# angelvillar96/STLPose

Hardware: AMD Instinct MI355X
Metric: images/sec/GPU HRNet-W32 384x288 train step; PCKh@0.5 parity (higher is better)
Workload: dtype f16/bf16; 1 GPU; HRNet-W32 384x288 bs=32/GPU train step (fwd+MSE+bwd+Adam), random-init weights; global_batch=32, parallelism=dp1

## Files before the change

### stlpose_amd/capi.py

```python
from __future__ import annotations

import ctypes as C
import os

import torch

from .cheader import Header

_HERE = os.path.dirname(os.path.abspath(__file__))
LIB_PATH = os.environ.get("STLPOSE_HIP_LIB") or os.path.join(_HERE, "libstlpose_hip.so")
INCLUDE = os.path.join(_HERE, "..", "include")
vp, i32, i64, f32 = C.c_void_p, C.c_int32, C.c_int64, C.c_float

CLASS_NAMES = {
    "stl_src": "Src", "stl_conv": "Conv", "stl_wgrad": "Wgrad", "stl_wgrad_io": "WgradIO", "stl_wgrad_group": "WgradGroup",
    "stl_term": "Term", "stl_fuse": "Fuse", "stl_fuse_bwd": "FuseBwd", "stl_upbwd": "UpBwd", "stl_wprep": "WPrep", "stl_slab": "Slab",
    "stl_bnrec": "BNRec", "stl_reduce_range": "ReduceRange", "stl_bn_range": "BNRange", "stl_patch": "Patch",
    "stl_patch_bwd": "PatchBwd", "stl_head": "Head", "stl_head_bwd": "HeadBwd", "stl_op": "Op", "StlDetImage": "DetImage",
    "StlDetPointwise": "DetPointwise", "StlDetTerm": "DetTerm", "StlDetFuse": "DetFuse", "StlDetPointwise16": "DetPointwise16",
    "StlDetPointwiseBwd": "DetPointwiseBwd", "StlDetPointwise16Bwd": "DetPointwise16Bwd"}
DEVICE_RECORDS = ("stl_wprep", "stl_slab", "stl_bnrec", "StlDetImage")

HEADER = Header(os.path.join(INCLUDE, "stlpose_hip.h"), CLASS_NAMES, DEVICE_RECORDS)
if set(HEADER.structs) != set(CLASS_NAMES):
    raise ImportError(f"capi.CLASS_NAMES and the structs of include/stlpose_hip.h differ: {sorted(set(HEADER.structs) ^ set(CLASS_NAMES))}")
globals().update({name[len("STL_"):]: value for name, value in HEADER.constants.items()})
globals().update({cls.__name__: cls for cls in HEADER.structs.values()})
SIGNATURES, RESTYPES = HEADER.signatures, HEADER.restypes
INT64_FUNCS = tuple(n for n, r in RESTYPES.items() if r is C.c_int64)
STRING_FUNCS = tuple(n for n, r in RESTYPES.items() if r is C.c_char_p)
DEBUG_SIGNATURES = Header(os.path.join(INCLUDE, "stlpose_hip_debug.h")).signatures
DETECTIONS = Header(os.path.join(INCLUDE, "stlpose_hip_detections.h"))

DTYPES = {F32: (4, torch.float32), BF16: (2, torch.bfloat16), F16: (2, torch.float16)}


def dt2(grad_dtype: int, fwd_dtype: int) -> int:
    return grad_dtype | ((fwd_dtype if fwd_dtype != grad_dtype else 0) << 8)


MIXED = dt2(BF16, F16)
POSE_APPROACH = {"all_kpts": POSE_ALL_KPTS, "full_body": POSE_FULL_BODY, "upper_body": POSE_UPPER_BODY}
POSE_DIM = {"all_kpts": 34, "full_body": 26, "upper_body": 18}
POSE_METHOD = {"euclidean": POSE_EUCLIDEAN, "cosine": POSE_COSINE, "manhattan": POSE_MANHATTAN, "confidence": POSE_CONFIDENCE,
               "oks": POSE_OKS, "l2sq": POSE_L2SQ, "cos_normalised": POSE_COS_NORMALISED}
POSE_PEN = {"zero_coord": POSE_PEN_ZERO_COORD, "none": POSE_PEN_NONE, "mean": POSE_PEN_MEAN, "max": POSE_PEN_MAX}
POSE_SUM_ORDER = {"numpy": POSE_SUM_NUMPY, "reference": POSE_SUM_SERIAL}
# ... 7 lines not shown

def lib() -> C.CDLL:
    global _lib
    if _lib is None:
        if not os.path.exists(LIB_PATH):
            raise RuntimeError(
                f"{LIB_PATH} not found: build it with `python -m stlpose_amd.build` "
                "(hipcc --offload-arch=gfx950). There is no CPU fallback for the product path.")
        l = C.CDLL(LIB_PATH)
        for name, args in SIGNATURES.items():
            fn = getattr(l, name)
            fn.argtypes, fn.restype = args, RESTYPES[name]
        for name, args in DETECTIONS.signatures.items():
            fn = getattr(l, name)
            fn.argtypes, fn.restype = args, DETECTIONS.restypes[name]
        for name, args in DEBUG_SIGNATURES.items():
            if hasattr(l, name):
                getattr(l, name).argtypes, getattr(l, name).restype = args, C.c_int
        _lib = l
    return _lib


def check(rc: int, what: str = "") -> None:
    if rc != 0:
        raise RuntimeError(f"stlpose_hip {what}: {lib().stl_last_error().decode()}")


def call(name: str, *args) -> None:
    check(getattr(lib(), name)(*args), name)
```

### stlpose_amd/csrc/elementwise.hip

```cpp
#include "common.cuh"

namespace {

template <typename T>
__device__ __forceinline__ void load8(const void* base, size_t elem, float* f) {
    if constexpr (sizeof(T) == 2) {
        unpack<T>(ldg16((const char*)base + elem * 2), f);
    } else {
        unpack<float>(ldg16((const char*)base + elem * 4), f);
        unpack<float>(ldg16((const char*)base + elem * 4 + 16), f + 4);
    }
}
template <typename T>
__device__ __forceinline__ void store8(void* base, size_t elem, const float* f) {
    if constexpr (sizeof(T) == 2) {
        stg16((char*)base + elem * 2, pack<T>(f));
    } else {
        stg16((char*)base + elem * 4, pack<float>(f));
        stg16((char*)base + elem * 4 + 16, pack<float>(f + 4));
    }
}

template <int NS>
__device__ __forceinline__ void flush_sets(float (*acc)[8], float* red, int C, int VPC, double* const* dst,
// ... 517 lines not shown

__global__ __launch_bounds__(256) void mse_kernel(const float* o, const float* t, const float* tw, float* dout,
                                                  double* partial, size_t n, int HW, float gs) {
    double acc = 0.0;
    for (size_t i = (size_t)blockIdx.x * 256 + threadIdx.x; i < n; i += (size_t)gridDim.x * 256) {
        const float w = tw[i / HW];
        const float d = (o[i] - t[i]) * w;
        acc += (double)d * (double)d;
        if (dout) dout[i] = d * w * gs;
    }
    __shared__ double sred[4];
    acc = wave_sum_d(acc);
    if ((threadIdx.x & 63) == 0) sred[threadIdx.x >> 6] = acc;
    __syncthreads();
    if (threadIdx.x == 0) partial[blockIdx.x] = sred[0] + sred[1] + sred[2] + sred[3];
}

__global__ __launch_bounds__(256) void sum_partials_kernel(const double* partial, int n, double scale, float* out, int accumulate) {
    double acc = 0.0;
    for (int i = threadIdx.x; i < n; i += 256) acc += partial[i];
    __shared__ double sred[4];
    acc = wave_sum_d(acc);
    if ((threadIdx.x & 63) == 0) sred[threadIdx.x >> 6] = acc;
    __syncthreads();
    if (threadIdx.x == 0) {
        const double s = (sred[0] + sred[1] + sred[2] + sred[3]) * scale;
        out[0] = (float)((accumulate ? (double)out[0] : 0.0) + s);
    }
}

// ... 89 lines not shown
    uint2 u;
    u.x = (uint32_t)__builtin_bit_cast(unsigned short, v[0]) | ((uint32_t)__builtin_bit_cast(unsigned short, v[1]) << 16);
    u.y = (uint32_t)__builtin_bit_cast(unsigned short, v[2]) | ((uint32_t)__builtin_bit_cast(unsigned short, v[3]) << 16);
    *reinterpret_cast<uint2*>(dst) = u;
}
__device__ __forceinline__ void store_vec4(f16* dst, const f16* v) {
    uint2 u;
    u.x = (uint32_t)__builtin_bit_cast(unsigned short, v[0]) | ((uint32_t)__builtin_bit_cast(unsigned short, v[1]) << 16);
    u.y = (uint32_t)__builtin_bit_cast(unsigned short, v[2]) | ((uint32_t)__builtin_bit_cast(unsigned short, v[3]) << 16);
    *reinterpret_cast<uint2*>(dst) = u;
}
__device__ __forceinline__ void store_vec4(float* dst, const float* v) {
    *reinterpret_cast<float4*>(dst) = make_float4(v[0], v[1], v[2], v[3]);
}

template <typename T, typename TF = T>
__global__ __launch_bounds__(256) void weight_prep_kernel(const float* master, T* wk, const stl_wprep* tab, int n, int blk_base) {
    static_assert(sizeof(T) == sizeof(TF), "both layouts live in one buffer of equal-width elements");
    TF* wkf = reinterpret_cast<TF*>(wk);
    const int bx = blockIdx.x + blk_base;
    const int ei = find_entry(&tab[0].blk0, sizeof(stl_wprep) / 4, n, bx);
    const stl_wprep e = tab[ei];
    const int t = e.ks * e.ks;
    const int64_t tot = (int64_t)e.Co * e.Ci * t;
    const int64_t base = (int64_t)(bx - e.blk0) * 1024;
    if (!e.patch && (e.Ci & 3) == 0 && (e.Co & 3) == 0 && t <= 9 && e.Cip == e.Ci && (e.fwd_off & 3) == 0 && (e.bwd_off < 0 || (e.bwd_off & 3) == 0)) {
        __shared__ float st[32 * (32 * 9 + 1)];
        const int pitch = 32 * t + 1;
        const int tci = (e.Ci + 31) >> 5, ntiles = ((e.Co + 31) >> 5) * tci;
        const int nblk = (int)((tot + 1023) / 1024);
        const float* src0 = master + e.src_off;
        for (int tile = bx - e.blk0; tile < ntiles; tile += nblk) {
            const int co0 = (tile / tci) * 32, ci0 = (tile % tci) * 32;
            const int nco = min(32, e.Co - co0), nci = min(32, e.Ci - ci0), seg = nci * t;
            __syncthreads();
            if (((e.src_off & 3) | (int)((uintptr_t)master & 15)) == 0) {
                const int nv = seg >> 2, ntask = nco * nv;
                float4 buf[9];
#pragma unroll
                for (int u = 0; u < 9; ++u) {
                    const int i = threadIdx.x + u * 256;
                    const bool ok = i < ntask;
                    const int r = ok ? i / nv : 0, q = ok ? i - r * nv : 0;
                    buf[u] = *reinterpret_cast<const float4*>(src0 + ((int64_t)(co0 + r) * e.Ci + ci0) * t + 4 * q);
                }
#pragma unroll
                for (int u = 0; u < 9; ++u) {
                    const int i = threadIdx.x + u * 256;
                    if (i < ntask) {
                        const int r = i / nv, q = i - r * nv;
                        float* d = st + r * pitch + 4 * q;
// ... 22 lines not shown
                for (int i = threadIdx.x; i < nci * t * p4; i += 256) {
                    const int row = p4 == 8 ? i >> 3 : i / p4, r4 = (i - row * p4) * 4;
                    const int c = t == 9 ? row / 9 : (t == 1 ? row : row / t), tapf = row - c * t;
#pragma unroll
                    for (int j = 0; j < 4; ++j) v[j] = (T)st[(r4 + j) * pitch + c * t + (t - 1 - tapf)];
                    store_vec4(wk + e.bwd_off + ((int64_t)(ci0 + c) * t + tapf) * e.Co + co0 + r4, v);
                }
            }
        }
        return;
    }
    for (int r = 0; r < 4; ++r) {
        const int64_t i = base + r * 256 + threadIdx.x;
        if (i >= tot) return;
        const int co = (int)(i / (e.Ci * t)), rem = (int)(i - (int64_t)co * e.Ci * t), ci = rem / t, tap = rem - ci * t;
        const float v = master[e.src_off + i];
        if (e.patch)
            wkf[e.fwd_off + (int64_t)co * e.Cip + tap * e.Ci + ci] = (TF)v;
        else
            wkf[e.fwd_off + ((int64_t)co * t + tap) * e.Cip + ci] = (TF)v;
        if (e.bwd_off >= 0) {
            if (e.patch)
                wk[e.bwd_off + (int64_t)(tap * e.Ci + ci) * e.Co + co] = (T)v;
            else
                wk[e.bwd_off + ((int64_t)ci * t + (t - 1 - tap)) * e.Co + co] = (T)v;
        }
    }
}

__global__ __launch_bounds__(256) void reduce_slabs_kernel(const float* partials, float* grads, const stl_slab* tab, int n, int blk_base) {
    const int bx = blockIdx.x + blk_base;
    const int ei = find_entry(&tab[0].blk0, sizeof(stl_slab) / 4, n, bx);
    const stl_slab e = tab[ei];
    const int t = e.ks * e.ks;
    const int64_t tot = (int64_t)e.Co * e.Ci * t;
    const int tk = e.patch ? 1 : t, cik = e.patch ? e.Cip : e.Ci;
    const int64_t slab = e.pad ? (int64_t)e.pad : (int64_t)e.Co * tk * cik;
    const int64_t base = (int64_t)(bx - e.blk0) * 1024;
    if (!e.patch && (e.Ci & 3) == 0) {
        const int64_t j = base + 4 * threadIdx.x;
        if (j >= tot) return;
        const float* src = partials + e.part_off + j;
// ... 80 lines not shown
            r1 += rstats[e.stats_off + (int64_t)k * 2 * e.C + c];
            r2 += rstats[e.stats_off + (int64_t)k * 2 * e.C + e.C + c];
        }
        grads[e.param_off + c] = (float)r2;
        grads[e.param_off + e.C + c] = (float)r1;
    }
}

__global__ void inc_step_kernel(int32_t* step, const int32_t* overflow) {
    const int t = step[0] < 0 ? -step[0] - 1 : step[0];
    step[0] = (overflow && overflow[0] != 0x7fffffff) ? -t - 1 : t + 1;
}

__global__ __launch_bounds__(256) void adam_kernel(float* p, const float* g, float* m, float* v, int64_t n,
                                                   const float* hyper, const int32_t* step) {
    const float lr = hyper[0], b1 = hyper[1], b2 = hyper[2], eps = hyper[3], wd = hyper[4], gs = hyper[7];
    const int t = step[0];
    if (t < 0) return;
    const float bc1 = 1.f - powf(b1, (float)t), bc2 = 1.f - powf(b2, (float)t);
    const float step_size = lr / bc1, isq2 = 1.f / sqrtf(bc2);
    for (int64_t i = (int64_t)blockIdx.x * 256 + threadIdx.x; i < n; i += (int64_t)gridDim.x * 256) {
        float gi = g[i] * gs;
        if (!(fabsf(gi) <= 3.4e38f)) continue;
        const float pi = p[i];
        if (wd != 0.f) gi = fmaf(wd, pi, gi);
        const float mi = b1 * m[i] + (1.f - b1) * gi;
        const float vi = b2 * v[i] + (1.f - b2) * gi * gi;
        m[i] = mi, v[i] = vi;
        p[i] = pi - step_size * mi / (sqrtf(vi) * isq2 + eps);
    }
}

__global__ __launch_bounds__(256) void sgd_kernel(float* p, const float* g, float* mom, int64_t n, const float* hyper,
                                                  const int32_t* step) {
    const float lr = hyper[0], wd = hyper[4], mu = hyper[5], nest = hyper[6], gs = hyper[7];
    if (step[0] < 0) return;
    const bool first = step[0] <= 1;
    for (int64_t i = (int64_t)blockIdx.x * 256 + threadIdx.x; i < n; i += (int64_t)gridDim.x * 256) {
        float gi = g[i] * gs;
        if (!(fabsf(gi) <= 3.4e38f)) continue;
        const float pi = p[i];
        if (wd != 0.f) gi = fmaf(wd, pi, gi);
        if (mu != 0.f) {
            const float b = first ? gi : mu * mom[i] + gi;
// ... 437 lines not shown
    STL_LAUNCH(sum_partials_kernel, dim3(1), dim3(256), 0, ST, partial, n, scale, out, accumulate);
    STL_LAUNCH_CHECK("sum_partials");
    return 0;
}

extern "C" int stl_mse_loss(const float* out, const float* target, const float* tweight, float* dout, double* partial,
                            int nblk, float* loss, int B, int J, int HW, float gscale, void* stream) {
    STL_CHECK(out && target && tweight && partial && nblk >= 1, "mse: null pointer");
    const size_t n = (size_t)B * J * HW;
    STL_LAUNCH(mse_kernel, dim3(nblk), dim3(256), 0, ST, out, target, tweight, dout, partial, n, HW, gscale / (float)n);
    STL_LAUNCH_CHECK("mse_loss");
    if (!loss) return 0;
    return stl_sum_partials(partial, nblk, 0.5 / (double)n, loss, 0, stream);
}

extern "C" int stl_heatmap_argmax(const float* hm, int32_t* idx, float* maxval, float* preds, int BJ, int H, int W, void* stream) {
    if (BJ == 0) return 0;
    STL_CHECK(hm && maxval && preds && H > 0 && W > 0, "argmax: bad args");
    STL_LAUNCH(argmax_kernel, dim3(BJ), dim3(256), 0, ST, hm, idx, maxval, preds, H, W);
    STL_LAUNCH_CHECK("heatmap_argmax");
    return 0;
}

extern "C" int stl_final_preds(const float* hm, const float* center, const float* scale, float* preds, float* maxval, int B,
                               int J, int H, int W, void* stream) {
    if (B * J == 0) return 0;
    STL_LAUNCH(final_preds_kernel, dim3(B * J), dim3(256), 0, ST, hm, center, scale, preds, maxval, J, H, W);
    STL_LAUNCH_CHECK("final_preds");
    return 0;
}
// ... 57 lines not shown
    return 0;
}

extern "C" int stl_bn_param_grads(const double* rstats, float* grads, const stl_bnrec* tab, int n, void* stream) {
    if (n == 0) return 0;
    STL_LAUNCH(bn_param_grads_kernel, dim3(n), dim3(256), 0, ST, rstats, grads, tab);
    STL_LAUNCH_CHECK("bn_param_grads");
    return 0;
}

extern "C" int stl_adam_step(float* p, const float* g, float* m, float* v, int64_t n, const float* hyper, int32_t* step, const int32_t* overflow,
                             void* stream) {
    STL_LAUNCH(inc_step_kernel, dim3(1), dim3(1), 0, ST, step, overflow);
    STL_LAUNCH(adam_kernel, dim3(nblocks_for((size_t)n, 256, 4096)), dim3(256), 0, ST, p, g, m, v, n, hyper, step);
    STL_LAUNCH_CHECK("adam_step");
    return 0;
}

extern "C" int stl_sgd_step(float* p, const float* g, float* mom, int64_t n, const float* hyper, int32_t* step, const int32_t* overflow, void* stream) {
    STL_LAUNCH(inc_step_kernel, dim3(1), dim3(1), 0, ST, step, overflow);
    STL_LAUNCH(sgd_kernel, dim3(nblocks_for((size_t)n, 256, 4096)), dim3(256), 0, ST, p, g, mom, n, hyper, step);
    STL_LAUNCH_CHECK("sgd_step");
    return 0;
}

__global__ __launch_bounds__(256) void gaussian_targets_kernel(const float* __restrict__ joints, const float* __restrict__ vis,
                                                               float* __restrict__ target, float* __restrict__ tw, int BJ, int Hh,
                                                               int Wh, double sx, double sy, float sigma) {
    const size_t total = (size_t)BJ * Hh * Wh;
    const float r = sigma * 3.f;
// ... 140 lines not shown
```

### stlpose_amd/engine.py

```python
from __future__ import annotations

import bisect
import ctypes as C
import math
import os
from dataclasses import dataclass, field
from typing import Dict, List, NamedTuple, Optional, Tuple, Union

import torch

from . import capi
from .arch import Arch, Registry, registry, walk

EPS = 1e-5
MOMENTUM = 0.1


def _esz(dtype: int) -> int:
    return capi.DTYPES[dtype & 0xff][0]


def choose_tile(B: int, Ho: int, Wo: int, stride: int, ks: int, esz: int, bn_cols: int = 64,
                maxpx: int = 128, maxhalo: int = 576) -> Tuple[int, int]:
    vrows = B * (Ho + 1)
# ... 162 lines not shown
        self.dtype, self.fdtype = dtype & 0xff, ((dtype >> 8) & 0xff) or (dtype & 0xff)
        self.ydtype = self.fdtype if self.fdtype != self.dtype else 0
        self.training = training
        self.input_grad = input_grad
        self.dev = store.device
        self.esz = _esz(dtype)
        self.tdtype = torch.float32 if self.dtype == capi.F32 else torch.bfloat16
        self.lib = capi.lib()
        self.fwd_ops: List[Launch] = []
        self.bwd_ops: List[Launch] = []
        self.tape: List[Union[ConvNode, FuseNode, HeadNode]] = []
        self.convs: List[ConvInfo] = []
        self.bns: List[BNInfo] = []
        self._keep: List = []
        self._progs: Dict[str, C.c_void_p] = {}
        self._fixups: Dict[str, List[Tuple]] = {}
        self.act_bytes = 0
        self.generation = 0
        self.img = torch.zeros(B, 3, H, W, dtype=torch.float32, device=self.dev)
        self.out: Optional[torch.Tensor] = None
        self.dout: Optional[torch.Tensor] = None
        self.dimg: Optional[torch.Tensor] = None
        nstat = bn_stat_elems(store.reg)
        self.stats = torch.zeros(max(nstat, 1), dtype=torch.float64, device=self.dev)
        self.rstats = torch.zeros(max(nstat, 1), dtype=torch.float64, device=self.dev) if training or input_grad else None
        self.sink = torch.zeros(max(nstat, 1), dtype=torch.float64, device=self.dev) if input_grad and not training else None
        self.overflow = torch.full((1,), 2 ** 31 - 1, dtype=torch.int32, device=self.dev)
        env = os.environ.get
        self.nstreams = int(env("STLPOSE_STREAMS", "4"))
        self.merge_minc = int(env("STLPOSE_MERGE_MINC", "128"))
# ... 484 lines not shown
        waits, need = self._schedule(ops, recorded)
        arr = (capi.Op * max(len(ops), 1))()
        for i, op in enumerate(ops):
            o = arr[i]
            o.kind, o.stream, o.desc = capi.OP_KIND[op.name], op.stream, C.addressof(op.desc)
            assert len(waits[i]) <= 8, "op waits on more than 8 producers"
            o.nwait = len(waits[i])
            for j, wv in enumerate(waits[i]):
                o.wait[j] = wv
            o.record = int(i in need)
        h = C.c_void_p()
        capi.call("stl_program_create", arr, len(ops), self.nstreams, C.byref(h))
        self._keep.append(arr)
        return h

    def _program(self, which: str) -> C.c_void_p:
        if which not in self._progs:
            self._progs[which] = (self._compile(self.fwd_ops, ()) if which == "fwd" else
                                  self._compile(self.bwd_ops, [b.op for b in self.buckets]))
        return self._progs[which]

    def _run(self, h, stream: int, on_bucket=None):
        if self._side is None:
            self._make_streams()
        self._stream_arr[0] = stream
        if on_bucket is None:
            if self.lib.stl_program_run(h, self._stream_arr) != 0:
                raise RuntimeError(f"stl_program_run: {self.lib.stl_last_error().decode()}")
            return
        first = 0
        for i, b in enumerate(self.buckets):
            capi.call("stl_program_run_range", h, self._stream_arr, first, b.op + 1)
            first = b.op + 1
            on_bucket(i)
        capi.call("stl_program_run_range", h, self._stream_arr, first, len(self.bwd_ops))

    def _make_streams(self):
        n = self.nstreams
        self._stream_arr = (C.c_void_p * n)()
        self._side = []
        pool = _STREAM_POOL.setdefault(self.dev.index, {})
        with torch.cuda.device(self.dev):
            for i in range(1, n):
                if i not in pool:
                    s_ = torch.cuda.Stream(device=self.dev)
                    pool[i] = (s_, s_.cuda_stream)
                self._side.append(pool[i][0])
                self._stream_arr[i] = pool[i][1]

    def prep_weights(self, stream: int):
        st = self.store
        capi.call("stl_weight_prep", capi.dt2(self.dtype, self.fdtype), st.master.data_ptr(), self.wk.data_ptr(), self._wprep_tab.data_ptr(),
                  self._wprep_n, self._wprep_blocks, stream)

    def forward(self, stream: int, update_running: bool = True):
        self.generation += 1
        self.prep_weights(stream)
        if self.training:
            self.stats.zero_()
        self._run(self._program("fwd"), stream)
        if self.training and update_running:
            st = self.store
            capi.call("stl_bn_running_update", self.stats.data_ptr(), st.bufs.data_ptr(), st.nbt.data_ptr(),
                      self._bn_tab.data_ptr(), len(self.bns), MOMENTUM, self.overflow.data_ptr(), stream)

    NO_OVERFLOW = 2 ** 31 - 1

    def check_forward_range(self):
        i = int(self.overflow.item())
        if i == self.NO_OVERFLOW:
            return
        self.overflow.fill_(self.NO_OVERFLOW)
        bn = self.bns[i]
        name = next((k for k, off in self.store.param_off.items() if off == bn.param_off), f"BatchNorm #{i}")
        what = {capi.F16: "f16 (|y| > 65504)", capi.BF16: "bf16", capi.F32: "fp32"}[self.fdtype]
        raise FloatingPointError(
            f"stlpose_amd: the raw output of the convolution in front of {name[:-len('.weight')] if name.endswith('.weight') else name} "
            f"left the range of its {what} storage (non-finite BatchNorm statistics; first such layer in forward order).  "
            "The optimiser skipped that step (and skips every step until this is reported): the weights are intact; the running "
            "statistics of the layers behind it took their momentum update from the poisoned pass.  Forward tensors of the default "
            "'mixed' mode are f16; for a checkpoint with badly scaled weights use compute_dtype='bf16' (same speed, bf16 range) "
            "or 'fp32'.")

    def backward(self, stream: int, on_bucket=None):
        assert self.training or self.input_grad
        if self.training:
            self.rstats.zero_()
        self._run(self._program("bwd"), stream, on_bucket if self.buckets else None)

    def bucket_wait(self, i: int, stream: int):
        capi.call("stl_program_wait_op", self._program("bwd"), self.buckets[i].op, stream)


_STREAM_POOL: Dict[int, Dict] = {}


def bn_weight_keys(reg: Registry) -> set:
    return {k[: -len("running_mean")] + "weight" for k, _ in reg.buffers if k.endswith("running_mean")}


def bn_stat_elems(reg: Registry) -> int:
    keys = bn_weight_keys(reg)
    return sum(int(math.prod(s)) for k, s in reg.params if k in keys) * 2 * capi.NSHARD


def _to_device(ctab, device) -> torch.Tensor:
    raw = bytes(ctab)
    t = torch.frombuffer(bytearray(raw), dtype=torch.uint8).clone()
    return t.to(device)
```

### stlpose_amd/train_step.py

```python
from __future__ import annotations

import os
from typing import List, Optional

import torch

from . import capi
from .dp import FlatAllReduce
from .hrnet import PoseHighResolutionNet

ADAM, SGD = "adam", "sgd"


class TrainStep:
    def __init__(self, model: PoseHighResolutionNet, batch: int, height: int, width: int, optimizer: str = ADAM,
                 lr: float = 1e-3, betas=(0.9, 0.999), eps: float = 1e-8, weight_decay: float = 0.0,
                 momentum: float = 0.9, nesterov: bool = False, process_group=None, bucket_mb: float = 32.0,
                 use_graph: bool = True, device=None, bf16_buckets: Optional[bool] = None):
        self.model = model
        from .hrnet import norm_device
        dev = norm_device(device or "cuda")
        if not model._packed(dev):
            model.to(dev)
            model._pack(dev)
        import weakref
        model._pinned_by = weakref.ref(self)
        model.train()
        self.dev = dev
        self.store = model._store
        self.eng = model.engine(batch, height, width, True)
        self.kind = optimizer
        self.pg = process_group
        if bf16_buckets is None:
            bf16_buckets = os.environ.get("STLPOSE_BF16_BUCKETS", "0") != "0"
# ... 22 lines not shown
        self.hyper = torch.tensor([lr, betas[0], betas[1], eps, weight_decay, momentum, float(nesterov), gscale],
                                  dtype=torch.float32, device=dev)
        self.step_count = torch.zeros(1, dtype=torch.int32, device=dev)
        J = self.eng.out.shape[1]
        self.target = torch.zeros_like(self.eng.out)
        self.tweight = torch.ones(batch, J, dtype=torch.float32, device=dev)
        self.loss = torch.zeros((), dtype=torch.float32, device=dev)
        self._nblk = 512
        self._partial = torch.zeros(self._nblk, dtype=torch.float64, device=dev)
        if self.eng.nstreams > 1:
            use_graph = False
        self.use_graph = use_graph
        self._g_fb: Optional[torch.cuda.CUDAGraph] = None
        self._g_opt: Optional[torch.cuda.CUDAGraph] = None
        self._loss_scale, self._loss_offset = 1.0, 0.0
        if self.use_graph and process_group is not None:
            self.use_graph = False

    def set_lr(self, lr: float):
        self.hyper[0] = lr

    def set_loss_affine(self, scale: float = 1.0, offset: float = 0.0):
        scale, offset = float(scale), float(offset)
        if self.use_graph and (scale, offset) != (self._loss_scale, self._loss_offset):
            self.use_graph = False
            self._g_fb = self._g_opt = None
        self._loss_scale, self._loss_offset = scale, offset

    def load_batch(self, img: torch.Tensor, target: torch.Tensor, target_weight: torch.Tensor):
        self.eng.img.copy_(img, non_blocking=True)
        self.target.copy_(target, non_blocking=True)
        self.tweight.copy_(target_weight.reshape(self.tweight.shape), non_blocking=True)

    def check_forward_range(self):
        self.eng.check_forward_range()

    def _fwd_bwd(self, update_running: bool = True):
        st = torch.cuda.current_stream().cuda_stream
        e = self.eng
        e.forward(st, update_running=update_running)
        B, J = e.out.shape[:2]
        HW = e.out[0, 0].numel()
        capi.call("stl_mse_loss", e.out.data_ptr(), self.target.data_ptr(), self.tweight.data_ptr(), e.dout.data_ptr(),
                  self._partial.data_ptr(), self._nblk, None, B, J, HW, self._loss_scale, st)
        dp_on = self.dp is not None and (self.world > 1 or self._force_dp) and not self.use_graph and self._dp_rccl
        e.backward(st, on_bucket=self._issue_bucket if dp_on else None)
        self._buckets_issued = dp_on
        capi.call("stl_sum_partials", self._partial.data_ptr(), self._nblk, 0.5 / float(B * J * HW), self.loss.data_ptr(), 0, st)
        if self._loss_scale != 1.0 or self._loss_offset != 0.0:
            self.loss.mul_(self._loss_scale).add_(self._loss_offset)

    def _optim(self):
        st = torch.cuda.current_stream().cuda_stream
        s = self.store
        if self.kind == ADAM:
            capi.call("stl_adam_step", s.master.data_ptr(), s.grads.data_ptr(), self.m.data_ptr(), self.v.data_ptr(),
                      s.nparam, self.hyper.data_ptr(), self.step_count.data_ptr(), self.eng.overflow.data_ptr(), st)
        else:
            capi.call("stl_sgd_step", s.master.data_ptr(), s.grads.data_ptr(), self.m.data_ptr(), s.nparam,
                      self.hyper.data_ptr(), self.step_count.data_ptr(), self.eng.overflow.data_ptr(), st)

    def _issue_bucket(self, i: int):
        if self._comm is None:
            self._comm = torch.cuda.Stream(device=self.dev)
        self.eng.bucket_wait(i, self._comm.cuda_stream)
        with torch.cuda.stream(self._comm):
            self.dp.launch(upto=i + 1, force=self._force_dp)

    def _allreduce(self):
        if self.dp is None or (self.world == 1 and not self._force_dp):
# ... 5 lines not shown

    def _capture(self):
        side = torch.cuda.Stream()
        side.wait_stream(torch.cuda.current_stream())
        with torch.cuda.stream(side):
            self._fwd_bwd(update_running=False)
        torch.cuda.current_stream().wait_stream(side)
        torch.cuda.synchronize()
        self._g_fb = torch.cuda.CUDAGraph()
        with torch.cuda.graph(self._g_fb):
            self._fwd_bwd()
        self._g_opt = torch.cuda.CUDAGraph()
        with torch.cuda.graph(self._g_opt):
            self._optim()

    def step(self) -> torch.Tensor:
        if self.use_graph:
            if self._g_fb is None:
                self._capture()
            self._g_fb.replay()
            self._allreduce()
            self._g_opt.replay()
        else:
            self._fwd_bwd()
            self._allreduce()
            self._optim()
        return self.loss
```

### stlpose_amd/trainer.py

```python
from __future__ import annotations

import json
import os
import time
from typing import Iterable, Optional

import numpy as np
import torch

from .hrnet import PoseHighResolutionNet, norm_device
from .inference import forward_pass
from .loss import PersonMSELoss, perceptual_affine
from .pose_parsing import accuracy
from .train_step import TrainStep

_PREFIX = "module."


def _timestamp() -> str:
    return time.strftime("%Y-%m-%d_%H-%M-%S")


def create_train_logs(exp_path: str) -> dict:
    logs = {"last_modified": _timestamp(), "iterations": 0,
# ... 65 lines not shown
                                                             step_size=int(tr["patience"]))
        else:
            self.scheduler = None
        if self.checkpoint is not None:
            self.load_checkpoint(self.checkpoint, only_model=not self.resume_training)
        self._broadcast_state()

    def _broadcast_state(self):
        if self.world == 1:
            return
        import torch.distributed as dist
        st, ts = self.ts.store, self.ts
        for t in (st.master, st.bufs, st.nbt, ts.m, ts.v, ts.step_count, ts.hyper):
            if t is not None:
                dist.broadcast(t, src=dist.get_global_rank(self.pg, 0), group=self.pg)

    def _mean_over_ranks(self, *vals):
        if self.world == 1:
            return vals
        import torch.distributed as dist
        t = torch.tensor(vals, dtype=torch.float64, device=self.device)
        dist.all_reduce(t, op=dist.ReduceOp.SUM, group=self.pg)
        return tuple((t / self.world).tolist())

    def _common_steps(self, loader) -> Optional[int]:
        if self.world == 1:
            return None
        import torch.distributed as dist
        try:
            n = len(loader)
# ... 154 lines not shown
```

Before: 2465 images/sec.

## Fuse Adam into weight-layout prep and fuse head conv with MSE loss backward

Merges the Adam update into the weight-prep kernel, so the optimizer writes the updated master weights straight into the low-precision compute layouts. This removes a separate full pass over the parameters and the prep pass at the start of forward; parameters not covered by conv weights are handled by extra remainder blocks. Separately, fuses the final 1x1 head conv forward, the MSE loss, its gradient, the input gradient and the head weight-grad partials into one kernel that uses MFMA. The cost is extra layout-stamp tracking to avoid stale layouts after external weight changes, plus more complex kernels.

Result: no change. 2463 images/sec (-0.1%).

```diff
diff --git a/include/stlpose_hip_train.h b/include/stlpose_hip_train.h
--- /dev/null
+++ b/include/stlpose_hip_train.h
@@ -0,0 +1,19 @@
+#ifndef STLPOSE_HIP_TRAIN_H
+#define STLPOSE_HIP_TRAIN_H
+#include <stdint.h>
+#ifdef __cplusplus
+extern "C" {
+#endif
+
+int stl_head_loss_backward(int dtype, const void* x, const float* w, const float* bias, const float* target,
+                           const float* tweight, float gscale, float* out, float* dout, double* lpartial, int npartial,
+                           void* dx, float* partial, int nblk, int B, int H, int W, int Ci, int J, void* stream);
+
+int stl_adam_prep_step(int dtype, float* p, const float* g, float* m, float* v, const float* hyper, int32_t* step,
+                       const int32_t* overflow , void* wk, const void* tab , int n, int nblocks,
+                       const int64_t* rem, int nrem, int64_t rem_total, void* stream);
+
+#ifdef __cplusplus
+}
+#endif
+#endif
diff --git a/stlpose_amd/capi.py b/stlpose_amd/capi.py
--- a/stlpose_amd/capi.py
+++ b/stlpose_amd/capi.py
@@ -31,6 +31,7 @@
 STRING_FUNCS = tuple(n for n, r in RESTYPES.items() if r is C.c_char_p)
 DEBUG_SIGNATURES = Header(os.path.join(INCLUDE, "stlpose_hip_debug.h")).signatures
 DETECTIONS = Header(os.path.join(INCLUDE, "stlpose_hip_detections.h"))
+TRAIN = Header(os.path.join(INCLUDE, "stlpose_hip_train.h"))
 
 DTYPES = {F32: (4, torch.float32), BF16: (2, torch.bfloat16), F16: (2, torch.float16)}
 
@@ -68,6 +69,9 @@
         for name, args in DETECTIONS.signatures.items():
             fn = getattr(l, name)
             fn.argtypes, fn.restype = args, DETECTIONS.restypes[name]
+        for name, args in TRAIN.signatures.items():
+            fn = getattr(l, name)
+            fn.argtypes, fn.restype = args, TRAIN.restypes[name]
         for name, args in DEBUG_SIGNATURES.items():
             if hasattr(l, name):
                 getattr(l, name).argtypes, getattr(l, name).restype = args, C.c_int
diff --git a/stlpose_amd/csrc/elementwise.hip b/stlpose_amd/csrc/elementwise.hip
--- a/stlpose_amd/csrc/elementwise.hip
+++ b/stlpose_amd/csrc/elementwise.hip
@@ -1,4 +1,5 @@
 #include "common.cuh"
+#include "../../include/stlpose_hip_train.h"
 
 namespace {
 
@@ -555,6 +556,150 @@
     if ((threadIdx.x & 63) == 0) sred[threadIdx.x >> 6] = acc;
     __syncthreads();
     if (threadIdx.x == 0) partial[blockIdx.x] = sred[0] + sred[1] + sred[2] + sred[3];
+}
+
+__device__ __forceinline__ void dd_add(double& hi, double& lo, double b, double blo) {
+    const double s = hi + b, bb = s - hi;
+    const double err = (hi - (s - bb)) + (b - bb);
+    hi = s, lo += err + blo;
+}
+template <typename T, int J, typename TY = T>
+__global__ __launch_bounds__(256) void head_loss_bwd_kernel(const void* x, const float* w, const float* bias, const float* target,
+                                                            const float* tw, float* out, float* dout, double* lpartial, void* dx,
+                                                            float* partial, int B, int HW, int Ci, float gs, int npartial) {
+    extern __shared__ __attribute__((aligned(16))) char smem[];
+    constexpr int SDP = 260;
+    constexpr int NTMAX = 4;
+    float* sw = reinterpret_cast<float*>(smem);
+    float* sd = sw + ((J * Ci + 3) & ~3);
+    float* sx = sd + J * SDP;
+    const int tid = threadIdx.x, lane = tid & 63, wave = tid >> 6, r16 = lane & 15, g = lane >> 4;
+    const int nt_n = Ci >> 4;
+    for (int e = tid; e < J * Ci; e += 256) sw[e] = w[e];
+    const int nel = J * Ci + J;
+    f32x4 acc[2][NTMAX];
+#pragma unroll
+    for (int mt = 0; mt < 2; ++mt)
+#pragma unroll
+        for (int nt = 0; nt < NTMAX; ++nt) acc[mt][nt] = f32x4{0.f, 0.f, 0.f, 0.f};
+    float bsum = 0.f;
+    double lacc = 0.0, lacc_lo = 0.0;
+    const size_t P = (size_t)B * HW;
+    const size_t nchunk = (P + 255) / 256;
+    for (size_t ch = blockIdx.x; ch < nchunk; ch += gridDim.x) {
+        const size_t pi = ch * 256 + tid;
+        __syncthreads();
+        float d[J];
+#pragma unroll
+        for (int j = 0; j < J; ++j) d[j] = bias ? bias[j] : 0.f;
+        for (int c0 = 0; c0 < Ci; c0 += 8) {
+            float f[8];
+            if (pi < P) {
+                load8<TY>(x, pi * Ci + c0, f);
+            } else {
+#pragma unroll
+                for (int q = 0; q < 8; ++q) f[q] = 0.f;
+            }
+#pragma unroll
+            for (int q = 0; q < 8; ++q) sx[tid * (Ci + 1) + c0 + q] = f[q];
+#pragma unroll
+            for (int j = 0; j < J; ++j)
+#pragma unroll
+                for (int q = 0; q < 8; ++q) d[j] = fmaf(f[q], sw[j * Ci + c0 + q], d[j]);
+        }
+        if (pi < P) {
+            const size_t b = pi / HW, hw = pi - b * HW;
+#pragma unroll
+            for (int j = 0; j < J; ++j) {
+                const size_t i = (b * J + j) * HW + hw;
+                const float wj = tw[b * J + j];
+                out[i] = d[j];
+                const float e = (d[j] - target[i]) * wj;
+                dd_add(lacc, lacc_lo, (double)e * (double)e, 0.0);
+                d[j] = e * wj * gs;
+                dout[i] = d[j];
+            }
+        } else {
+#pragma unroll
+            for (int j = 0; j < J; ++j) d[j] = 0.f;
+        }
+#pragma unroll
+        for (int j = 0; j < J; ++j) sd[j * SDP + tid] = d[j];
+        for (int c0 = 0; c0 < Ci; c0 += 8) {
+            float gx[8];
+#pragma unroll
+            for (int q = 0; q < 8; ++q) {
+                float s = 0.f;
+#pragma unroll
+                for (int j = 0; j < J; ++j) s = fmaf(d[j], sw[j * Ci + c0 + q], s);
+                gx[q] = s;
+            }
+            if (pi < P) store8<T>(dx, pi * Ci + c0, gx);
+        }
+        __syncthreads();
+        const int px0 = wave * 64 + g;
+        const float* arow0 = sd + r16 * SDP + px0;
+        const float* arow1 = sd + (16 + r16 < J ? 16 + r16 : 0) * SDP + px0;
+        const bool a1ok = 16 + r16 < J;
+        const float* brow = sx + (size_t)px0 * (Ci + 1) + r16;
+#pragma unroll 4
+        for (int ks = 0; ks < 16; ++ks) {
+            const float a0 = arow0[4 * ks];
+            const float a1 = a1ok ? arow1[4 * ks] : 0.f;
+#pragma unroll
+            for (int nt = 0; nt < NTMAX; ++nt) {
+                if (nt < nt_n) {
+                    const float bv = brow[(size_t)4 * ks * (Ci + 1) + nt * 16];
+                    acc[0][nt] = __builtin_amdgcn_mfma_f32_16x16x4f32(a0, bv, acc[0][nt], 0, 0, 0);
+                    acc[1][nt] = __builtin_amdgcn_mfma_f32_16x16x4f32(a1, bv, acc[1][nt], 0, 0, 0);
+                }
+            }
+        }
+        if (tid < 4 * J) {
+            const float* r = sd + (tid >> 2) * SDP + (tid & 3) * 64;
+            float s = 0.f;
+#pragma unroll
+            for (int q = 0; q < 16; ++q) {
+                const float4 v = *reinterpret_cast<const float4*>(r + 4 * q);
+                s += (v.x + v.y) + (v.z + v.w);
+            }
+            bsum += s;
+        }
+    }
+    __shared__ double sred[8];
+#pragma unroll
+    for (int o = 32; o > 0; o >>= 1) dd_add(lacc, lacc_lo, __shfl_xor(lacc, o), __shfl_xor(lacc_lo, o));
+    if (lane == 0) sred[2 * wave] = lacc, sred[2 * wave + 1] = lacc_lo;
+    __syncthreads();
+    if (tid == 0) {
+        double hi = sred[0], lo = sred[1];
+        for (int k = 1; k < 4; ++k) dd_add(hi, lo, sred[2 * k], sred[2 * k + 1]);
+        lpartial[2 * blockIdx.x] = hi, lpartial[2 * blockIdx.x + 1] = lo;
+    }
+    if (blockIdx.x == 0)
+        for (int k = 2 * gridDim.x + tid; k < npartial; k += 256) lpartial[k] = 0.0;
+    f32x4* red = reinterpret_cast<f32x4*>(sx);
+#pragma unroll
+    for (int mt = 0; mt < 2; ++mt)
+#pragma unroll
+        for (int nt = 0; nt < NTMAX; ++nt)
+            if (nt < nt_n) red[(wave * 2 * NTMAX + mt * NTMAX + nt) * 64 + lane] = acc[mt][nt];
+    float* bred = reinterpret_cast<float*>(red + 4 * 2 * NTMAX * 64);
+    if (tid < 4 * J) bred[tid] = bsum;
+    __syncthreads();
+    for (int e = tid; e < nel; e += 256) {
+        float s;
+        if (e < J * Ci) {
+            const int j = e / Ci, c = e - j * Ci;
+            const int tile = (j >> 4) * NTMAX + (c >> 4), ln = 16 * ((j & 15) >> 2) + (c & 15), rr = j & 3;
+            s = (red[(0 * 2 * NTMAX + tile) * 64 + ln][rr] + red[(1 * 2 * NTMAX + tile) * 64 + ln][rr]) +
+                (red[(2 * 2 * NTMAX + tile) * 64 + ln][rr] + red[(3 * 2 * NTMAX + tile) * 64 + ln][rr]);
+        } else {
+            const int j = e - J * Ci;
+            s = (bred[4 * j] + bred[4 * j + 1]) + (bred[4 * j + 2] + bred[4 * j + 3]);
+        }
+        partial[(size_t)blockIdx.x * nel + e] = s;
+    }
 }
 
 __global__ __launch_bounds__(256) void sum_partials_kernel(const double* partial, int n, double scale, float* out, int accumulate) {
@@ -674,10 +819,77 @@
     *reinterpret_cast<float4*>(dst) = make_float4(v[0], v[1], v[2], v[3]);
 }
 
-template <typename T, typename TF = T>
-__global__ __launch_bounds__(256) void weight_prep_kernel(const float* master, T* wk, const stl_wprep* tab, int n, int blk_base) {
+struct adam_consts {
+    float b1, b2, eps, wd, gs, step_size, isq2;
+    bool on;
+};
+__device__ __forceinline__ adam_consts adam_setup(const float* hyper, const int32_t* step) {
+    adam_consts c;
+    const float lr = hyper[0];
+    c.b1 = hyper[1], c.b2 = hyper[2], c.eps = hyper[3], c.wd = hyper[4], c.gs = hyper[7];
+    const int t = step[0];
+    c.on = t >= 0;
+    const float bc1 = 1.f - powf(c.b1, (float)t), bc2 = 1.f - powf(c.b2, (float)t);
+    c.step_size = lr / bc1, c.isq2 = 1.f / sqrtf(bc2);
+    return c;
+}
+__device__ __forceinline__ bool adam_update(const adam_consts& c, float& p, float g, float& m, float& v) {
+#pragma clang fp contract(off)
+    float gi = g * c.gs;
+    if (!(fabsf(gi) <= 3.4e38f)) return false;
+    const float pi = p;
+    if (c.wd != 0.f) gi = fmaf(c.wd, pi, gi);
+    const float mg = (1.f - c.b1) * gi;
+    const float mi = fmaf(c.b1, m, mg);
+    const float vi = c.b2 * v + (1.f - c.b2) * gi * gi;
+    m = mi, v = vi;
+    p = pi - c.step_size * mi / (sqrtf(vi) * c.isq2 + c.eps);
+    return true;
+}
+__device__ __forceinline__ void adam_update4(const adam_consts& c, float4& p, const float4& g, float4& m, float4& v) {
+    adam_update(c, p.x, g.x, m.x, v.x);
+    adam_update(c, p.y, g.y, m.y, v.y);
+    adam_update(c, p.z, g.z, m.z, v.z);
+    adam_update(c, p.w, g.w, m.w, v.w);
+}
+
+struct adam_prep_args {
+    const float* g;
+    float* m;
+    float* v;
+    const float* hyper;
+    const int32_t* step;
+    const int64_t* rem;
+    int64_t rem_total;
+    int nrem, nprep_blocks;
+};
+
+template <typename T, typename TF, bool OPT>
+__device__ __forceinline__ void weight_prep_body(std::conditional_t<OPT, float, const float>* master, T* wk, const stl_wprep* tab,
+                                                 int n, int blk_base, const adam_prep_args& a) {
     static_assert(sizeof(T) == sizeof(TF), "both layouts live in one buffer of equal-width elements");
     TF* wkf = reinterpret_cast<TF*>(wk);
+    adam_consts ac;
+    if constexpr (OPT) {
+        ac = adam_setup(a.hyper, a.step);
+        if ((int)blockIdx.x >= a.nprep_blocks) {
+            if (!ac.on) return;
+            const int64_t k0 = (int64_t)(blockIdx.x - a.nprep_blocks) * 1024;
+            for (int r = 0; r < 4; ++r) {
+                const int64_t k = k0 + r * 256 + threadIdx.x;
+                if (k >= a.rem_total) return;
+                int lo = 0, hi = a.nrem - 1;
+                while (lo < hi) {
+                    const int mid = (lo + hi + 1) >> 1;
+                    if (a.rem[2 * mid + 1] <= k) lo = mid; else hi = mid - 1;
+                }
+                const int64_t i = a.rem[2 * lo] + (k - a.rem[2 * lo + 1]);
+                float pi = master[i], mi = a.m[i], vi = a.v[i];
+                if (adam_update(ac, pi, a.g[i], mi, vi)) master[i] = pi, a.m[i] = mi, a.v[i] = vi;
+            }
+            return;
+        }
+    }
     const int bx = blockIdx.x + blk_base;
     const int ei = find_entry(&tab[0].blk0, sizeof(stl_wprep) / 4, n, bx);
     const stl_wprep e = tab[ei];
@@ -694,7 +906,53 @@
             const int co0 = (tile / tci) * 32, ci0 = (tile % tci) * 32;
             const int nco = min(32, e.Co - co0), nci = min(32, e.Ci - ci0), seg = nci * t;
             __syncthreads();
-            if (((e.src_off & 3) | (int)((uintptr_t)master & 15)) == 0) {
+            if constexpr (OPT) {
+                if (((e.src_off & 3) | (int)(((uintptr_t)master | (uintptr_t)a.g | (uintptr_t)a.m | (uintptr_t)a.v) & 15)) == 0) {
+                    const int nv = seg >> 2, ntask = nco * nv;
+                    for (int u0 = 0; u0 < 9 && u0 * 256 < ntask; u0 += 3) {
+                        float4 bp[3], bg[3], bm[3], bv[3];
+                        int64_t off[3];
+#pragma unroll
+                        for (int k = 0; k < 3; ++k) {
+                            const int i = threadIdx.x + (u0 + k) * 256;
+                            const bool ok = i < ntask;
+                            const int r = ok ? i / nv : 0, q = ok ? i - r * nv : 0;
+                            off[k] = e.src_off + ((int64_t)(co0 + r) * e.Ci + ci0) * t + 4 * q;
+                            bp[k] = *reinterpret_cast<const float4*>(master + off[k]);
+                            bg[k] = *reinterpret_cast<const float4*>(a.g + off[k]);
+                            bm[k] = *reinterpret_cast<const float4*>(a.m + off[k]);
+                            bv[k] = *reinterpret_cast<const float4*>(a.v + off[k]);
+                        }
+#pragma unroll
+                        for (int k = 0; k < 3; ++k) {
+                            const int i = threadIdx.x + (u0 + k) * 256;
+                            if (i < ntask) {
+                                if (ac.on) {
+                                    adam_update4(ac, bp[k], bg[k], bm[k], bv[k]);
+                                    *reinterpret_cast<float4*>(master + off[k]) = bp[k];
+                                    *reinterpret_cast<float4*>(a.m + off[k]) = bm[k];
+                                    *reinterpret_cast<float4*>(a.v + off[k]) = bv[k];
+                                }
+                                const int r = i / nv, q = i - r * nv;
+                                float* d = st + r * pitch + 4 * q;
+                                d[0] = bp[k].x, d[1] = bp[k].y, d[2] = bp[k].z, d[3] = bp[k].w;
+                            }
+                        }
+                    }
+                } else {
+                    for (int r = threadIdx.x >> 6; r < nco; r += 4) {
+                        const int64_t row = e.src_off + ((int64_t)(co0 + r) * e.Ci + ci0) * t;
+                        for (int c = threadIdx.x & 63; c < seg; c += 64) {
+                            float pi = master[row + c];
+                            if (ac.on) {
+                                float mi = a.m[row + c], vi = a.v[row + c];
+                                if (adam_update(ac, pi, a.g[row + c], mi, vi)) master[row + c] = pi, a.m[row + c] = mi, a.v[row + c] = vi;
+                            }
+                            st[r * pitch + c] = pi;
+                        }
+                    }
+                }
+            } else if (((e.src_off & 3) | (int)((uintptr_t)master & 15)) == 0) {
                 const int nv = seg >> 2, ntask = nco * nv;
                 float4 buf[9];
 #pragma unroll
@@ -747,7 +1005,14 @@
         const int64_t i = base + r * 256 + threadIdx.x;
         if (i >= tot) return;
         const int co = (int)(i / (e.Ci * t)), rem = (int)(i - (int64_t)co * e.Ci * t), ci = rem / t, tap = rem - ci * t;
-        const float v = master[e.src_off + i];
+        float v = master[e.src_off + i];
+        if constexpr (OPT) {
+            if (ac.on) {
+                const int64_t k = e.src_off + i;
+                float mi = a.m[k], vi = a.v[k];
+                if (adam_update(ac, v, a.g[k], mi, vi)) master[k] = v, a.m[k] = mi, a.v[k] = vi;
+            }
+        }
         if (e.patch)
             wkf[e.fwd_off + (int64_t)co * e.Cip + tap * e.Ci + ci] = (TF)v;
         else
@@ -759,6 +1024,15 @@
                 wk[e.bwd_off + ((int64_t)ci * t + (t - 1 - tap)) * e.Co + co] = (T)v;
         }
     }
+}
+
+template <typename T, typename TF = T>
+__global__ __launch_bounds__(256) void weight_prep_kernel(const float* master, T* wk, const stl_wprep* tab, int n, int blk_base) {
+    weight_prep_body<T, TF, false>(master, wk, tab, n, blk_base, adam_prep_args{});
+}
+template <typename T, typename TF = T>
+__global__ __launch_bounds__(256) void adam_kernel_prep(float* master, T* wk, const stl_wprep* tab, int n, const adam_prep_args a) {
+    weight_prep_body<T, TF, true>(master, wk, tab, n, 0, a);
 }
 
 __global__ __launch_bounds__(256) void reduce_slabs_kernel(const float* partials, float* grads, const stl_slab* tab, int n, int blk_base) {
@@ -869,20 +1143,11 @@
 
 __global__ __launch_bounds__(256) void adam_kernel(float* p, const float* g, float* m, float* v, int64_t n,
                                                    const float* hyper, const int32_t* step) {
-    const float lr = hyper[0], b1 = hyper[1], b2 = hyper[2], eps = hyper[3], wd = hyper[4], gs = hyper[7];
-    const int t = step[0];
-    if (t < 0) return;
-    const float bc1 = 1.f - powf(b1, (float)t), bc2 = 1.f - powf(b2, (float)t);
-    const float step_size = lr / bc1, isq2 = 1.f / sqrtf(bc2);
+    const adam_consts c = adam_setup(hyper, step);
+    if (!c.on) return;
     for (int64_t i = (int64_t)blockIdx.x * 256 + threadIdx.x; i < n; i += (int64_t)gridDim.x * 256) {
-        float gi = g[i] * gs;
-        if (!(fabsf(gi) <= 3.4e38f)) continue;
-        const float pi = p[i];
-        if (wd != 0.f) gi = fmaf(wd, pi, gi);
-        const float mi = b1 * m[i] + (1.f - b1) * gi;
-        const float vi = b2 * v[i] + (1.f - b2) * gi * gi;
-        m[i] = mi, v[i] = vi;
-        p[i] = pi - step_size * mi / (sqrtf(vi) * isq2 + eps);
+        float pi = p[i], mi = m[i], vi = v[i];
+        if (adam_update(c, pi, g[i], mi, vi)) m[i] = mi, v[i] = vi, p[i] = pi;
     }
 }
 
@@ -1350,6 +1615,42 @@
     return stl_sum_partials(partial, nblk, 0.5 / (double)n, loss, 0, stream);
 }
 
+extern "C" int stl_head_loss_backward(int dtype2, const void* x, const float* w, const float* bias, const float* target,
+                                      const float* tweight, float gscale, float* out, float* dout, double* lpartial, int npartial,
+                                      void* dx, float* partial, int nblk, int B, int H, int W, int Ci, int J, void* stream) {
+    const int dtype = dtype2 & 0xff, ydtype = (dtype2 >> 8) & 0xff;
+    STL_CHECK(x && w && target && tweight && out && dout && lpartial && dx && partial, "head_loss_bwd: null pointer");
+    STL_CHECK(ydtype == 0 || ydtype == dtype || (dtype == STL_BF16 && ydtype == STL_F16), "head_loss_bwd: x type %d does not go with dx type %d", ydtype, dtype);
+    STL_CHECK(dtype == STL_F32 || dtype == STL_BF16, "head_loss_bwd: dx type %d", dtype);
+    STL_CHECK(J == 17 || J == 16, "head_loss_bwd: J=%d unsupported", J);
+    STL_CHECK(Ci % 16 == 0 && Ci <= 64, "head_loss_bwd: Ci=%d must be a multiple of 16, at most 64", Ci);
+    STL_CHECK(B >= 1 && H >= 1 && W >= 1, "head_loss_bwd: empty tensor");
+    STL_CHECK(nblk >= 1 && 2 * nblk <= npartial, "head_loss_bwd: %d blocks need %d loss partials, not %d", nblk, 2 * nblk, npartial);
+    size_t lds = (size_t)(((J * Ci + 3) & ~3) + J * 260 + 256 * (Ci + 1)) * 4;
+    const size_t lds_red = (size_t)(((J * Ci + 3) & ~3) + J * 260) * 4 + (size_t)4 * 2 * 4 * 64 * 16 + 4 * J * 4;
+    if (lds_red > lds) lds = lds_red;
+    static bool attr = false;
+    constexpr int kMaxLds = 159 * 1024;
+    if (!attr) {
+        hipFuncSetAttribute(reinterpret_cast<const void*>(&head_loss_bwd_kernel<__bf16, 17>), hipFuncAttributeMaxDynamicSharedMemorySize, kMaxLds);
+        hipFuncSetAttribute(reinterpret_cast<const void*>(&head_loss_bwd_kernel<__bf16, 16>), hipFuncAttributeMaxDynamicSharedMemorySize, kMaxLds);
+        hipFuncSetAttribute(reinterpret_cast<const void*>(&head_loss_bwd_kernel<float, 17>), hipFuncAttributeMaxDynamicSharedMemorySize, kMaxLds);
+        hipFuncSetAttribute(reinterpret_cast<const void*>(&head_loss_bwd_kernel<float, 16>), hipFuncAttributeMaxDynamicSharedMemorySize, kMaxLds);
+        hipFuncSetAttribute(reinterpret_cast<const void*>(&head_loss_bwd_kernel<__bf16, 17, f16>), hipFuncAttributeMaxDynamicSharedMemorySize, kMaxLds);
+        hipFuncSetAttribute(reinterpret_cast<const void*>(&head_loss_bwd_kernel<__bf16, 16, f16>), hipFuncAttributeMaxDynamicSharedMemorySize, kMaxLds);
+        attr = true;
+    }
+    const size_t n = (size_t)B * J * H * W;
+    const float gs = gscale / (float)n;
+#define HLB(T, JJ, TY) STL_LAUNCH((head_loss_bwd_kernel<T, JJ, TY>), dim3(nblk), dim3(256), lds, ST, x, w, bias, target, tweight, out, dout, lpartial, dx, partial, B, H * W, Ci, gs, npartial)
+    if (dtype == STL_BF16 && ydtype == STL_F16) { if (J == 17) HLB(__bf16, 17, f16); else HLB(__bf16, 16, f16); }
+    else if (dtype == STL_BF16) { if (J == 17) HLB(__bf16, 17, __bf16); else HLB(__bf16, 16, __bf16); }
+    else { if (J == 17) HLB(float, 17, float); else HLB(float, 16, float); }
+#undef HLB
+    STL_LAUNCH_CHECK("head_loss_backward");
+    return 0;
+}
+
 extern "C" int stl_heatmap_argmax(const float* hm, int32_t* idx, float* maxval, float* preds, int BJ, int H, int W, void* stream) {
     if (BJ == 0) return 0;
     STL_CHECK(hm && maxval && preds && H > 0 && W > 0, "argmax: bad args");
@@ -1437,6 +1738,31 @@
     STL_LAUNCH(inc_step_kernel, dim3(1), dim3(1), 0, ST, step, overflow);
     STL_LAUNCH(adam_kernel, dim3(nblocks_for((size_t)n, 256, 4096)), dim3(256), 0, ST, p, g, m, v, n, hyper, step);
     STL_LAUNCH_CHECK("adam_step");
+    return 0;
+}
+
+extern "C" int stl_adam_prep_step(int dtype2, float* p, const float* g, float* m, float* v, const float* hyper, int32_t* step,
+                                  const int32_t* overflow, void* wk, const void* tabv, int n, int nblocks, const int64_t* rem,
+                                  int nrem, int64_t rem_total, void* stream) {
+    const stl_wprep* tab = static_cast<const stl_wprep*>(tabv);
+    STL_CHECK(p && g && m && v && hyper && step && wk && tab && n > 0 && nblocks > 0, "adam_prep: bad arguments");
+    STL_CHECK(nrem >= 0 && rem_total >= 0 && (nrem == 0) == (rem_total == 0) && (nrem == 0 || rem), "adam_prep: bad remainder table");
+    const int dtype = dtype2 & 0xff, fdtype = (dtype2 >> 8) & 0xff;
+    STL_CHECK(fdtype == 0 || fdtype == dtype || (dtype == STL_BF16 && fdtype == STL_F16), "adam_prep: forward type %d does not go with %d", fdtype, dtype);
+    const int64_t rblocks = (rem_total + 1023) / 1024;
+    STL_CHECK(nblocks + rblocks < (int64_t)1 << 31, "adam_prep: too many blocks");
+    const adam_prep_args a{g, m, v, hyper, step, rem, rem_total, nrem, nblocks};
+    const dim3 grid((unsigned)(nblocks + rblocks));
+    STL_LAUNCH(inc_step_kernel, dim3(1), dim3(1), 0, ST, step, overflow);
+    if (dtype == STL_BF16 && fdtype == STL_F16)
+        STL_LAUNCH((adam_kernel_prep<__bf16, f16>), grid, dim3(256), 0, ST, p, (__bf16*)wk, tab, n, a);
+    else if (dtype == STL_F16)
+        STL_LAUNCH((adam_kernel_prep<f16, f16>), grid, dim3(256), 0, ST, p, (f16*)wk, tab, n, a);
+    else if (dtype == STL_BF16)
+        STL_LAUNCH((adam_kernel_prep<__bf16, __bf16>), grid, dim3(256), 0, ST, p, (__bf16*)wk, tab, n, a);
+    else
+        STL_LAUNCH((adam_kernel_prep<float, float>), grid, dim3(256), 0, ST, p, (float*)wk, tab, n, a);
+    STL_LAUNCH_CHECK("adam_prep_step");
     return 0;
 }
 
diff --git a/stlpose_amd/engine.py b/stlpose_amd/engine.py
--- a/stlpose_amd/engine.py
+++ b/stlpose_amd/engine.py
@@ -200,6 +200,8 @@
         self.bns: List[BNInfo] = []
         self._keep: List = []
         self._progs: Dict[str, C.c_void_p] = {}
+        self._bwd_head = True
+        self._adam_rem = None
         self._fixups: Dict[str, List[Tuple]] = {}
         self.act_bytes = 0
         self.generation = 0
@@ -714,13 +716,21 @@
         self._keep.append(arr)
         return h
 
-    def _program(self, which: str) -> C.c_void_p:
+    def _program(self, which: str, head: bool = True) -> C.c_void_p:
+        if not head:
+            assert self.fwd_ops[-1].name == "stl_head_forward" and self.bwd_ops[0].name == "stl_head_backward"
+            assert all(b.op >= 1 for b in self.buckets)
+            key = which + "-head"
+            if key not in self._progs:
+                self._progs[key] = (self._compile(self.fwd_ops[:-1], ()) if which == "fwd" else
+                                    self._compile(self.bwd_ops[1:], [b.op - 1 for b in self.buckets]))
+            return self._progs[key]
         if which not in self._progs:
             self._progs[which] = (self._compile(self.fwd_ops, ()) if which == "fwd" else
                                   self._compile(self.bwd_ops, [b.op for b in self.buckets]))
         return self._progs[which]
 
-    def _run(self, h, stream: int, on_bucket=None):
+    def _run(self, h, stream: int, on_bucket=None, skip: int = 0):
         if self._side is None:
             self._make_streams()
         self._stream_arr[0] = stream
@@ -730,10 +740,10 @@
             return
         first = 0
         for i, b in enumerate(self.buckets):
-            capi.call("stl_program_run_range", h, self._stream_arr, first, b.op + 1)
-            first = b.op + 1
+            capi.call("stl_program_run_range", h, self._stream_arr, first, b.op + 1 - skip)
+            first = b.op + 1 - skip
             on_bucket(i)
-        capi.call("stl_program_run_range", h, self._stream_arr, first, len(self.bwd_ops))
+        capi.call("stl_program_run_range", h, self._stream_arr, first, len(self.bwd_ops) - skip)
 
     def _make_streams(self):
         n = self.nstreams
@@ -753,12 +763,36 @@
         capi.call("stl_weight_prep", capi.dt2(self.dtype, self.fdtype), st.master.data_ptr(), self.wk.data_ptr(), self._wprep_tab.data_ptr(),
                   self._wprep_n, self._wprep_blocks, stream)
 
-    def forward(self, stream: int, update_running: bool = True):
+    def adam_prep_step(self, m: torch.Tensor, v: torch.Tensor, hyper: torch.Tensor, step: torch.Tensor, stream: int):
+        st = self.store
+        assert self._adam_rem is not None, "plan_adam_prep() first"
+        rem, nrem, rtotal = self._adam_rem
+        capi.call("stl_adam_prep_step", capi.dt2(self.dtype, self.fdtype), st.master.data_ptr(), st.grads.data_ptr(), m.data_ptr(),
+                  v.data_ptr(), hyper.data_ptr(), step.data_ptr(), self.overflow.data_ptr(), self.wk.data_ptr(),
+                  self._wprep_tab.data_ptr(), self._wprep_n, self._wprep_blocks, rem.data_ptr(), nrem, rtotal, stream)
+
+    def plan_adam_prep(self):
+        st = self.store
+        if self._adam_rem is None:
+            rem = adam_remainder([(c.master_off, c.Co * c.Ci * c.ks * c.ks) for c in self.convs], st.nparam)
+            flat, before = [], 0
+            for lo, hi in rem:
+                flat += [lo, before]
+                before += hi - lo
+            self._adam_rem = (torch.tensor(flat or [0, 0], dtype=torch.int64, device=self.dev), len(rem), before)
+
+    def head_loss_backward(self, target: torch.Tensor, tweight: torch.Tensor, gscale: float, partial: torch.Tensor, stream: int):
+        hd, hb = self.fwd_ops[-1].desc, self.bwd_ops[0].desc
+        capi.call("stl_head_loss_backward", hb.dtype, hb.x, hb.w, hd.bias, target.data_ptr(), tweight.data_ptr(), gscale, hd.out,
+                  hb.dout, partial.data_ptr(), partial.numel(), hb.dx, hb.partial, hb.nblk, hb.B, hb.H, hb.W, hb.Ci, hb.J, stream)
+
+    def forward(self, stream: int, update_running: bool = True, prep: bool = True, head: bool = True):
         self.generation += 1
-        self.prep_weights(stream)
+        if prep:
+            self.prep_weights(stream)
         if self.training:
             self.stats.zero_()
-        self._run(self._program("fwd"), stream)
+        self._run(self._program("fwd", head), stream)
         if self.training and update_running:
             st = self.store
             capi.call("stl_bn_running_update", self.stats.data_ptr(), st.bufs.data_ptr(), st.nbt.data_ptr(),
@@ -782,14 +816,16 @@
             "'mixed' mode are f16; for a checkpoint with badly scaled weights use compute_dtype='bf16' (same speed, bf16 range) "
             "or 'fp32'.")
 
-    def backward(self, stream: int, on_bucket=None):
+    def backward(self, stream: int, on_bucket=None, head: bool = True):
         assert self.training or self.input_grad
         if self.training:
             self.rstats.zero_()
-        self._run(self._program("bwd"), stream, on_bucket if self.buckets else None)
+        self._bwd_head = head
+        self._run(self._program("bwd", head), stream, on_bucket if self.buckets else None, skip=0 if head else 1)
 
     def bucket_wait(self, i: int, stream: int):
-        capi.call("stl_program_wait_op", self._program("bwd"), self.buckets[i].op, stream)
+        head = self._bwd_head
+        capi.call("stl_program_wait_op", self._program("bwd", head), self.buckets[i].op - (0 if head else 1), stream)
 
 
 _STREAM_POOL: Dict[int, Dict] = {}
@@ -797,6 +833,21 @@
 
 def bn_weight_keys(reg: Registry) -> set:
     return {k[: -len("running_mean")] + "weight" for k, _ in reg.buffers if k.endswith("running_mean")}
+
+
+def adam_remainder(ranges: List[Tuple[int, int]], nparam: int) -> List[Tuple[int, int]]:
+    rem, at = [], 0
+    for off, size in sorted(ranges):
+        if size <= 0 or off < at or off + size > nparam:
+            raise ValueError(f"adam_remainder: conv weight [{off}, {off + size}) overlaps its predecessor (ending at {at}) "
+                             f"or leaves the parameter buffer [0, {nparam})")
+        if off > at:
+            rem.append((at, off))
+        at = off + size
+    if at < nparam:
+        rem.append((at, nparam))
+    assert sum(s for _, s in ranges) + sum(hi - lo for lo, hi in rem) == nparam
+    return rem
 
 
 def bn_stat_elems(reg: Registry) -> int:
diff --git a/stlpose_amd/train_step.py b/stlpose_amd/train_step.py
--- a/stlpose_amd/train_step.py
+++ b/stlpose_amd/train_step.py
@@ -16,8 +16,9 @@
     def __init__(self, model: PoseHighResolutionNet, batch: int, height: int, width: int, optimizer: str = ADAM,
                  lr: float = 1e-3, betas=(0.9, 0.999), eps: float = 1e-8, weight_decay: float = 0.0,
                  momentum: float = 0.9, nesterov: bool = False, process_group=None, bucket_mb: float = 32.0,
-                 use_graph: bool = True, device=None, bf16_buckets: Optional[bool] = None):
+                 use_graph: bool = True, device=None, bf16_buckets: Optional[bool] = None, fused: bool = True):
         self.model = model
+        self.fused = fused
         from .hrnet import norm_device
         dev = norm_device(device or "cuda")
         if not model._packed(dev):
@@ -70,6 +71,11 @@
         self._g_fb: Optional[torch.cuda.CUDAGraph] = None
         self._g_opt: Optional[torch.cuda.CUDAGraph] = None
         self._loss_scale, self._loss_offset = 1.0, 0.0
+        self._prep_in_forward = not (fused and optimizer == ADAM)
+        if not self._prep_in_forward:
+            self.eng.plan_adam_prep()
+        self._params = [p for p in model.parameters()]
+        self._layouts_of: Optional[int] = None
         if self.use_graph and process_group is not None:
             self.use_graph = False
 
@@ -94,13 +100,18 @@
     def _fwd_bwd(self, update_running: bool = True):
         st = torch.cuda.current_stream().cuda_stream
         e = self.eng
-        e.forward(st, update_running=update_running)
+        if not torch.cuda.is_current_stream_capturing():
+            self._ensure_layouts()
+        e.forward(st, update_running=update_running, prep=self._prep_in_forward, head=not self.fused)
         B, J = e.out.shape[:2]
         HW = e.out[0, 0].numel()
-        capi.call("stl_mse_loss", e.out.data_ptr(), self.target.data_ptr(), self.tweight.data_ptr(), e.dout.data_ptr(),
-                  self._partial.data_ptr(), self._nblk, None, B, J, HW, self._loss_scale, st)
+        if self.fused:
+            e.head_loss_backward(self.target, self.tweight, self._loss_scale, self._partial, st)
+        else:
+            capi.call("stl_mse_loss", e.out.data_ptr(), self.target.data_ptr(), self.tweight.data_ptr(), e.dout.data_ptr(),
+                      self._partial.data_ptr(), self._nblk, None, B, J, HW, self._loss_scale, st)
         dp_on = self.dp is not None and (self.world > 1 or self._force_dp) and not self.use_graph and self._dp_rccl
-        e.backward(st, on_bucket=self._issue_bucket if dp_on else None)
+        e.backward(st, on_bucket=self._issue_bucket if dp_on else None, head=not self.fused)
         self._buckets_issued = dp_on
         capi.call("stl_sum_partials", self._partial.data_ptr(), self._nblk, 0.5 / float(B * J * HW), self.loss.data_ptr(), 0, st)
         if self._loss_scale != 1.0 or self._loss_offset != 0.0:
@@ -109,7 +120,9 @@
     def _optim(self):
         st = torch.cuda.current_stream().cuda_stream
         s = self.store
-        if self.kind == ADAM:
+        if self.kind == ADAM and self.fused:
+            self.eng.adam_prep_step(self.m, self.v, self.hyper, self.step_count, st)
+        elif self.kind == ADAM:
             capi.call("stl_adam_step", s.master.data_ptr(), s.grads.data_ptr(), self.m.data_ptr(), self.v.data_ptr(),
                       s.nparam, self.hyper.data_ptr(), self.step_count.data_ptr(), self.eng.overflow.data_ptr(), st)
         else:
@@ -145,10 +158,25 @@
         with torch.cuda.graph(self._g_opt):
             self._optim()
 
+    def _layout_stamp(self) -> int:
+        return self.store.master._version + sum(p._version for p in self._params)
+
+    def _ensure_layouts(self):
+        if self._prep_in_forward:
+            return
+        stamp = self._layout_stamp()
+        if self._layouts_of != stamp:
+            self.eng.prep_weights(torch.cuda.current_stream().cuda_stream)
+            self._layouts_of = stamp
+
+    def invalidate_layouts(self):
+        self._layouts_of = None
+
     def step(self) -> torch.Tensor:
         if self.use_graph:
             if self._g_fb is None:
                 self._capture()
+            self._ensure_layouts()
             self._g_fb.replay()
             self._allreduce()
             self._g_opt.replay()
diff --git a/stlpose_amd/trainer.py b/stlpose_amd/trainer.py
--- a/stlpose_amd/trainer.py
+++ b/stlpose_amd/trainer.py
@@ -103,6 +103,7 @@
         for t in (st.master, st.bufs, st.nbt, ts.m, ts.v, ts.step_count, ts.hyper):
             if t is not None:
                 dist.broadcast(t, src=dist.get_global_rank(self.pg, 0), group=self.pg)
+        ts.invalidate_layouts()
 
     def _mean_over_ranks(self, *vals):
         if self.world == 1:
```
